# NickDrake117/GNNkeras

Measured on AMD Instinct MI355X. Metric: node-state updates/s (arcs x iterations / s), forward Loop, higher is better.
Workload: dtype f32; 1 GPU; C4 Erdos-Renyi 1000000 nodes / 10000000 arcs, state_dim=64, max_iteration=50, threshold=0 (k=50), node-focused, average aggregation, BN+Dense(159->64,selu) state net

## Files before the change

### gnnkeras_amd/csrc/gnnloop.hip

```cpp
#include <hip/hip_runtime.h>
#include <stdarg.h>
#include <stddef.h>
#include <stdio.h>
#include <stdlib.h>
#include <string.h>
#include <algorithm>
#include <mutex>
#include <string>
#include <vector>

#include "../../include/gnnloop.h"
#include "kernels_general.hpp"
#include "kernel_state_fused2.hpp"
#include "kernel_state_fused4.hpp"
#include "kernel_state_small.hpp"
#include "kernel_state_mid.hpp"
#include "kernel_state_lds.hpp"
#include "kernel_state_lds_types.hpp"
#include "kernel_state_wide.hpp"
#include "kernels_batch.hpp"
#include "kernels_setup.hpp"
#include "kernel_rowdense.hpp"
#include "kernel_state_xwide.hpp"

// ... 32 lines not shown
int state_ld(int S) {
    if (S <= 128) {
        int p = 16;
        while (p < S) p <<= 1;
        return p;
    }
    return round_up(S, 4);
}

struct Knobs {
    int pin;
    int flag_pin, env_pin;
    int mid_max_nodes;
    bool prefix_fusion, xwide, rowdense;
    bool xc; int xc_min_nodes;
};
const Knobs &process_knobs() {
    static const Knobs once = [] {
        Knobs k = {};
        const char *e;
        k.env_pin = (e = getenv("GNN_FUSED_KERNEL")) ? atoi(e) : 0;
        k.mid_max_nodes = (e = getenv("GNN_MID_MAX_NODES")) ? atoi(e) : 36000;
        k.prefix_fusion = !((e = getenv("GNN_PREFIX_FUSION")) && e[0] == '0');
        k.xwide = !((e = getenv("GNN_XWIDE")) && atoi(e) == 0);
        k.rowdense = !((e = getenv("GNN_ROWDENSE")) && e[0] == '0');
        return k;
    }();
    return once;
}
Knobs knobs(int flags) {
    Knobs k = process_knobs();
    k.flag_pin = (flags & GNN_FLAG_FUSED_GEN_MASK) >> 4;
    k.pin = k.flag_pin ? k.flag_pin : k.env_pin;
    const char *e = getenv("GNN_XC"), *m = getenv("GNN_XC_MIN_NODES");
    k.xc = !(e && atoi(e) == 0);
    k.xc_min_nodes = m ? atoi(m) : 196608;
    return k;
}

struct Carver {
    char *base;
    size_t off = 0;
    explicit Carver(void *b) : base((char *)b) {}
    template <typename T>
    T *take(size_t count) {
        off = (off + 255) & ~(size_t)255;
        T *p = base ? (T *)(base + off) : nullptr;
        off += count * sizeof(T);
        return p;
    }
};
// ... 306 lines not shown
    int count;
    float *Wf, *bf;
    float *Wc;
    int wrow_state, wrow_agg;
    gnn::Seg cseg[GNN_MAX_SEGS];
    int ncseg;
};

struct Plan {
    int N, E, S, SP, L, A, T;
    int H1max, Hmax_state, Hmax_out, Tout, M, G;
    bool composite, fused;
    int n_heavy;
    TypePlan tp[GNN_MAX_TYPES];
    int *flags;
    int *mid_bar;
    gnn::GroupTab gt;
    int n_groups;
    int group_tiles;
    int group_max_nodes;
    int *d_group_tabs;
    unsigned long long *set_bar;
    bool has_sets;
    int *pred0;
    int *tbeg;
    int *err;
    float *agg_arcs, *agg_nodes; int ld_agg_nodes;
    float *C; int ldC;
    float *Xc;
    float *Wx;
// ... 102 lines not shown
            TRY(check_csr(a.nodegraph, "nodegraph", a.nodegraph.n_dst, p.M));
        }
        if (a.n_heavy_segments > 0) {
            if (!a.heavy_seg_beg || !a.heavy_seg_end) return fail("heavy_seg_beg / heavy_seg_end is NULL");
            TRY(check_csr(a.adjacency_light, "adjacency_light", p.N, (a.nodes_src ? a.adjacency.n_src : p.N) + a.n_heavy_segments));
        }
        if (p.composite) {
            if (!a.type_nodes && p.N > 0) return fail("type_nodes is NULL");
            if (a.type_offsets[0] != 0 || a.type_offsets[p.T] != p.N) return fail("type_offsets must span [0, n_nodes]");
            for (int t = 0; t < p.T; ++t)
                TRY(check_csr(a.composite_adjacency[t], "composite_adjacency", p.N, a.nodes_src ? a.adjacency.n_src : p.N));
        }
    }

    Carver c(ws);
    p.flags = c.take<int>(a.max_iteration + GNN_LOOP_WORDS);
    p.err = p.flags ? p.flags + a.max_iteration + 12 : nullptr;
    p.mid_bar = p.flags ? p.flags + ((a.max_iteration + 16 + 31) & ~31) : nullptr;
    p.pred0 = c.take<int>(std::max(GNN_SMALL_MAX_TILES, p.group_tiles));
    p.d_group_tabs = c.take<int>(a.n_groups > 0 ? 4 * ((size_t)a.n_groups + 1) : 0);
    p.set_bar = c.take<unsigned long long>(a.n_groups > 0 ? 2 * (size_t)a.n_groups : 0);
    for (int t = 0; t < p.T; ++t) {
        p.tp[t].Wf = c.take<float>((size_t)a.net_state[t].in_dim * a.net_state[t].units[0]);
        p.tp[t].bf = c.take<float>(a.net_state[t].units[0]);
    }
    p.Wf_out = c.take<float>((size_t)a.net_output.in_dim * a.net_output.units[0]);
    p.bf_out = c.take<float>(a.net_output.units[0]);
    p.agg_arcs = c.take<float>((size_t)p.N * std::max(p.A, 1));
    p.ld_agg_nodes = p.composite ? sum_dt : (a.state_dim > 0 ? p.L : 0);
    p.agg_nodes = c.take<float>((size_t)p.N * std::max(p.ld_agg_nodes, 1));
    p.ldC = (p.H1max + 3) & ~3;
// ... 40 lines not shown
                if (p.A > 0) tp.cseg[tp.ncseg++] = gnn::Seg{p.agg_arcs, nullptr, p.A, p.A, 2 * p.S};
            }
        } else {
            const int dt = a.type_dim_label[t];
            tp.rows = a.type_nodes ? a.type_nodes + a.type_offsets[t] : nullptr;
            tp.count = a.type_offsets[t + 1] - a.type_offsets[t];
            tp.wrow_state = dt; tp.wrow_agg = dt + p.S;
            if (dt > 0) tp.cseg[tp.ncseg++] = gnn::Seg{a.nodes, tp.rows, a.ld_nodes, dt, 0};
            if (sum_dt > 0) tp.cseg[tp.ncseg++] = gnn::Seg{p.agg_nodes, tp.rows, p.ld_agg_nodes, sum_dt, dt + 2 * p.S};
            if (p.A > 0) tp.cseg[tp.ncseg++] = gnn::Seg{p.agg_arcs, tp.rows, p.A, p.A, dt + 2 * p.S + sum_dt};
        }
    }
    return 0;
}

inline const gnn_csr_t &iter_adjacency(const gnn_loop_args_t &a, const Plan &p) { return p.n_heavy > 0 ? a.adjacency_light : a.adjacency; }

}
#include "loop_route.hpp"
namespace {

int launch_heavy(const gnn_loop_args_t &a, const Plan &p, const int *gate, const float *src, hipStream_t st) {
    if (p.n_heavy == 0) return 0;
    float *buf = const_cast<float *>(src);
    const int first_virtual = a.nodes_src ? a.adjacency.n_src : p.N;
    const int grid = std::min(p.n_heavy, 256 * 8);
    switch (p.SP) {
        case 16: gnn::k_heavy_segments<16><<<grid, 256, 0, st>>>(gate, a.heavy_seg_beg, a.heavy_seg_end, p.n_heavy, a.adjacency.src, a.adjacency.w, buf, first_virtual); break;
        case 32: gnn::k_heavy_segments<32><<<grid, 256, 0, st>>>(gate, a.heavy_seg_beg, a.heavy_seg_end, p.n_heavy, a.adjacency.src, a.adjacency.w, buf, first_virtual); break;
        case 64: gnn::k_heavy_segments<64><<<grid, 256, 0, st>>>(gate, a.heavy_seg_beg, a.heavy_seg_end, p.n_heavy, a.adjacency.src, a.adjacency.w, buf, first_virtual); break;
// ... 43 lines not shown
    LAUNCH_OK();
    return 0;
}
int check_xc_args(const gnn_loop_args_t &a) {
    if (!a.xc) return 0;
    if (((uintptr_t)a.xc & 255) != 0) return fail("xc must be 256-byte aligned");
    if (a.xc_mode != GNN_XC_FILL && a.xc_mode != GNN_XC_VALID) return fail("unknown xc_mode %d", a.xc_mode);
    return 0;
}

int setup_constants(const gnn_loop_args_t &a, const Plan &p, hipStream_t st, bool zero_loop_words = false, bool skip_c = false,
                    const GivenAgg *given = nullptr, bool xc_line = false, bool xc_valid = false) {
    FoldList fl;
    for (int t = 0; t < p.T; ++t) fl.add(a.net_state[t], p.tp[t].Wf, p.tp[t].bf);
    if (a.net_output.kernel[0]) fl.add(a.net_output, p.Wf_out, p.bf_out);
    if (zero_loop_words) { fl.fa.zero_a = p.flags; fl.fa.n_a = a.max_iteration + GNN_LOOP_WORDS; fl.fa.zero_b = a.k_out; fl.fa.n_b = 1; }
    TRY(launch_fold_list(fl, st));
    if (xc_line) {
        const TypePlan &tp = p.tp[0];
        if (!xc_valid) TRY(fill_constants_line(a, p.N, a.state_dim > 0 ? p.L : 0, p.A, p.Xc, st));
        gnn::PackSegs ps;
        memset(&ps, 0, sizeof(ps));
        ps.n = tp.ncseg;
        for (int s2 = 0; s2 < tp.ncseg && s2 < 3; ++s2) { ps.width[s2] = tp.cseg[s2].width; ps.wrow[s2] = tp.cseg[s2].wrow; }
        const int H = tp.net->units[0];
        gnn::k_pack_wc<<<cdiv(32 * H, 256), 256, 0, st>>>(tp.Wf, tp.bf, H, ps, tp.Wc);
        LAUNCH_OK();
        return 0;
    }
    if (given) {
        if (p.A > 0) TRY(launch_copy2d(nullptr, given->arcs, given->ld_arcs, p.agg_arcs, p.A, p.N, p.A, p.A, st));
// ... 53 lines not shown
    const int L = a.state_dim > 0 ? p.L : 0;
    sa.N = p.N; sa.n_tiles = p.group_tiles; sa.groups = p.gt;
    if (p.n_groups > GNN_MAX_GROUPS || (p.n_groups > 0 && p.gt.n == 0)) {
        sa.groups.d_node_begin = p.d_group_tabs; sa.groups.d_tile_begin = p.d_group_tabs + (p.n_groups + 1); sa.groups.n_dev = p.n_groups;
    }
    sa.nodes = a.nodes; sa.ld_nodes = a.ld_nodes; sa.L = L;
    sa.nodes_src = a.nodes_src ? a.nodes_src : a.nodes; sa.ld_nodes_src = a.nodes_src ? a.ld_nodes_src : a.ld_nodes;
    sa.adj = gnn::SetupCsr{a.adjacency.rowptr, a.adjacency.src, a.adjacency.w, a.adjacency.row_scale};
    sa.arc_labels = a.arc_labels; sa.ld_arcs = a.ld_arcs; sa.A = p.A;
    sa.arcnode = gnn::SetupCsr{a.arcnode.rowptr, a.arcnode.src, a.arcnode.w, a.arcnode.row_scale};
    if (a.state_dim > 0) { sa.row_nodes = p.S; sa.row_aggn = 2 * p.S + p.L; sa.row_agga = 2 * p.S + 2 * p.L; }
    else                 { sa.row_agga = 2 * p.S; }
    sa.C = p.C; sa.ldC = p.ldC;
    sa.state0 = a.state_dim > 0 ? a.state0 : a.nodes; sa.ld_s0 = a.state_dim > 0 ? p.S : a.ld_nodes;
    sa.S = p.S; sa.thr = a.state_threshold; sa.pred0 = p.pred0;
    sa.zero_a = p.flags; sa.n_a = a.max_iteration + GNN_LOOP_WORDS; sa.zero_b = a.k_out; sa.n_b = std::max(1, p.n_groups);
    gnn::k_setup_small<<<sa.n_tiles + 1, 256, gnn::setup_small_lds(sa.net.H, 2 * L + p.A, std::max(a.net_state[0].in_dim, a.net_output.in_dim)), st>>>(sa);
    LAUNCH_OK();
    return 0;
}

__global__ void k_fold_error(const int *err, float *k_out) {
    if (*err != 0) *k_out = -1.0e9f;
}

int launch_fold_error(const Plan &p, float *k_out, hipStream_t st) {
    if (!k_out || !p.err) return 0;
    k_fold_error<<<1, 1, 0, st>>>(p.err, k_out);
    LAUNCH_OK();
    return 0;
}
// ... 83 lines not shown
    r.nseg = 1;
    r.segs[0] = gnn::Seg{p.agg, nullptr, p.SP, (int)m.units[1], 0};
    r.M = p.N;
    r.hid[0] = p.hid[0]; r.hid[1] = p.hid[1]; r.ld_hid = p.ld_hid;
    r.Y = dst; r.ldy = p.SP;
    r.gate = gate;
    if (flag_next) { r.pred_old = src; r.ld_pred = p.SP; r.pred_thr = a.state_threshold; r.pred_flag = flag_next; r.pred_k = k_out; r.pred_kval = k_val; }
    TRY(run_mlp(r, st));
    if (flag_next && !r.pred_fused) TRY(launch_converge(gate, dst, src, p.N, p.S, p.SP, p.SP, a.state_threshold, flag_next, k_out, k_val, st));
    return 0;
}

int iteration_fused(const gnn_loop_args_t &a, const Plan &p, IterKernel kernel, const int *gate, int n_gate, int gate_stride,
                    const float *src, float *dst, int row_base, int *flag_next, float *k_out, float k_val,
                    hipStream_t st, const gnn_csr_t *adj_override = nullptr, const float *agg_init = nullptr,
                    const int *rows_override = nullptr, int count_override = 0, const gnn_peer_set_t *peers = nullptr) {
    TRY(launch_heavy(a, p, n_gate == 1 ? gate : nullptr, src, st));
    const gnn_csr_t &adj = adj_override ? *adj_override : iter_adjacency(a, p);
    gnn::Fused2Args fa;
    memset(&fa, 0, sizeof(fa));
    fill_fused_args(fa, a, p, adj);
    fa.gate = n_gate ? gate : nullptr; fa.n_gate = n_gate; fa.gate_stride = gate_stride;
    fa.state_in = src; fa.state_out = dst; fa.row_base = row_base; fa.err = p.err;
    if (rows_override && fa.n_types == 1) {
        fa.tp[0].rows = rows_override; fa.tp[0].count = count_override;
        if (count_override == 0) fa.n_types = 0;
    }
    fa.flag_next = flag_next;
    fa.k_out = k_out; fa.k_val = k_val;
    fa.agg_init = agg_init;
    if (peers) {
        if (peers->n_peers < 0 || peers->n_peers > GNN_MAX_PEERS) return fail("n_peers %d out of [0, %d]", peers->n_peers, GNN_MAX_PEERS);
        fa.n_peers = peers->n_peers;
        for (int i = 0; i < peers->n_peers; ++i) fa.peer_out[i] = peers->state_out_full[i];
    }
    if (p.xc_ok && !adj.w && (agg_init || size_generation(p, a.flags) == 4)) fa.Xc = p.Xc;
    if (fa.n_types == 0) {
        if (k_out) TRY(launch_converge(fa.gate, src, src, 0, p.S, p.SP, p.SP, a.state_threshold, flag_next, k_out, k_val, st));
        return 0;
    }
    if (fa.n_peers > 0 && (p.SP == 128 || p.T != 1 || adj.w || a.net_state[0].n_layers != 1 || (p.SP != 32 && p.SP != 64) || p.n_heavy != 0))
        return fail("peer stores: homogeneous one-layer shards without per-arc weights or hub rows, state widths 17 .. 64");
    if (kernel == IterKernel::wide) FUSED_OK(gnn::launch_wide(fa, device_cus(), st, 0));
    else if (kernel == IterKernel::fused4 || agg_init || fa.n_peers > 0) FUSED_OK(gnn::launch_fused4(fa, p.SP, device_cus(), st));
    else FUSED_OK(gnn::launch_fused2(fa, p.SP, 8, device_cus(), st));
// ... 224 lines not shown
        for (int t = 0; t <= GNN_MAX_TYPES; ++t) to.off[t] = a.type_offsets[std::min(t, p.T)];
        gnn::k_group_type_begin<<<cdiv(p.T * (p.n_groups + 1), 256), 256, 0, st>>>(a.type_nodes, to, p.T, p.d_group_tabs, p.n_groups, p.tbeg);
        LAUNCH_OK();
        gnn::k_pred0_groups<<<p.n_groups, 256, 0, st>>>(p.d_group_tabs, a.state_dim > 0 ? a.state0 : a.nodes, a.state_dim > 0 ? p.S : a.ld_nodes, p.S,
                                                        a.state_threshold, p.pred0);
        LAUNCH_OK();
        if (a.ev_loop_begin) HIP_OK(hipEventRecord((hipEvent_t)a.ev_loop_begin, st));
        const int rc = loop_lds_types(a, p, st);
        if (rc != 0) return rc == 2 ? fail("LDS-resident loop kernel does not cover these convergence groups") : 1;
        if (a.ev_loop_end) HIP_OK(hipEventRecord((hipEvent_t)a.ev_loop_end, st));
        return output_stage(a, p, st);
    }
    default: break;
    }
    const bool small_setup = route.small_setup, xc_loop = route.xc_loop, xc_line = route.xc_line;
    if (xc_line && a.xc) { TRY(check_xc_args(a)); p.Xc = a.xc; }
    if (small_setup) TRY(setup_small(a, p, st));
    else             TRY(setup_constants(a, p, st, true, xc_loop, nullptr, xc_line,
                                         xc_line && a.xc && a.xc_mode == GNN_XC_VALID));

    const float *first = p.buf[0];
    if (a.state_dim > 0 && p.S == p.SP && p.n_heavy == 0 && (reinterpret_cast<uintptr_t>(a.state0) & 15) == 0) first = a.state0;
    else if (a.state_dim > 0) TRY(launch_copy2d(nullptr, a.state0, p.S, p.buf[0], p.SP, p.N, p.S, p.SP, st));
    else                      TRY(launch_copy2d(nullptr, a.nodes, a.ld_nodes, p.buf[0], p.SP, p.N, p.S, p.SP, st));
    if (p.SP != p.S) HIP_OK(hipMemsetAsync(p.buf[1], 0, sizeof(float) * (size_t)p.N * p.SP, st));
    if (!small_setup) TRY(launch_converge(nullptr, first, nullptr, p.N, p.S, p.SP, 0, a.state_threshold, p.flags, nullptr, 0.f, st));

    const IterKernel kernel = route.iter.kernel;
    if (kernel == IterKernel::xwide) TRY(setup_xwide(a, p, st));
    const bool no_exit = (a.flags & GNN_FLAG_NO_EARLY_EXIT) != 0;
// ... 5 lines not shown
    if (route.whole == WholeLoop::small) {
        persistent = loop_whole(a, p, false, first, B, small_setup ? p.pred0 : nullptr, small_setup ? p.group_tiles : 0, a.state_out, st);
        if (persistent == 1) return 1;
        if (persistent == 2 && small_setup) return fail("whole-loop kernel refused a graph its set-up kernel accepted");
    }
    bool loop_done = persistent == 0;
    if (!loop_done && route.try_mid) {
        const int rc = loop_whole(a, p, true, first, B, nullptr, 0, nullptr, st);
        if (rc == 1) return 1;
        loop_done = rc == 0;
    }
    for (int it = 0; !loop_done && it < a.max_iteration; ++it) {
        const int *gate = no_exit ? nullptr : p.flags + it;
        const float *src = it == 0 ? first : B[it & 1];
        float *dst = B[(it + 1) & 1];
        if (route.iter.fused())                  TRY(iteration_fused(a, p, kernel, gate, gate ? 1 : 0, 0, src, dst, 0, p.flags + it + 1, a.k_out, (float)(it + 1), st));
        else if (kernel == IterKernel::prefix)   TRY(iteration_prefix(a, p, gate, src, dst, p.flags + it + 1, a.k_out, (float)(it + 1), st));
        else if (kernel == IterKernel::xwide)    TRY(iteration_xwide(a, p, gate, src, dst, p.flags + it + 1, a.k_out, (float)(it + 1), st));
        else                                     TRY(iteration_unfused(a, p, gate, src, dst, 0, p.flags + it + 1, a.k_out, (float)(it + 1), st));
    }

    if (a.ev_loop_end) HIP_OK(hipEventRecord((hipEvent_t)a.ev_loop_end, st));

    if (persistent != 0) {
        const long total = (long)p.N * p.S;
        if (total > 0) {
            gnn::k_select_state<<<std::min(cdiv(total, 256), 256 * 16), 256, 0, st>>>(a.k_out, first, B[0], B[1], p.SP, a.state_out, p.S, p.N, p.S);
            LAUNCH_OK();
        }
    }
    TRY(output_stage(a, p, st));
// ... 433 lines not shown
```

### gnnkeras_amd/csrc/kernel_state_fused2.hpp

```cpp
#pragma once
#include <hip/hip_runtime.h>
#include "kernels_general.hpp"

namespace gnn {

struct FusedType {
    const int *rows;
    int count;
    const float *Wf;
    int wrow_state, wrow_agg;
    int H, act;
    const float *W2;
    const float *b2;
    int act2;
    const float *Wc;
    int out2;
};

struct Fused2Args {
    const int *gate; int n_gate, gate_stride;
    const int *rowptr, *src;
    const float *w, *row_scale;
    const float *state_in;
    float *state_out;
    int row_base;
    const float *C; int ldC;
    int n_types;
    FusedType tp[GNN_MAX_TYPES];
    int blk_begin[GNN_MAX_TYPES + 1];
    int S;
    float thr;
    int *flag_next;
    float *k_out; float k_val;
    int *err;
    const float *Xc;
    const float *agg_init;
    const void *hdr; void *hdr_write;
    float *peer_out[GNN_MAX_PEERS]; int n_peers;
};

inline char *last_kernel_name() { static thread_local char name[96] = ""; return name; }
#define GNN_SET_KERNEL_NAME(...) snprintf(::gnn::last_kernel_name(), 96, __VA_ARGS__)

template <int SP, int TM, int NW>
struct Fused2Cfg {
    static constexpr int NT = 64 * NW;
    static constexpr int LPR = SP / 4;
    static constexpr int NPP = NT / LPR;
    static constexpr int NPASS = TM / NPP;
    static constexpr int IPL = 16 / LPR;
    static constexpr int LDX = 2 * SP + 2;
    static constexpr bool SWZ = SP >= 32;
    static constexpr int LDW = SWZ ? SP : SP + 32;
// ... 319 lines not shown
```

### gnnkeras_amd/csrc/kernel_state_fused4.hpp

```cpp
#pragma once
#include <hip/hip_runtime.h>
#include "kernel_state_fused2.hpp"
#include "buffer_ops.hpp"

namespace gnn {

constexpr int XC_K = 32;

template <int SP, int NC = 4, bool L2 = false, bool XC = false, int VPL = 1>
struct Fused4Cfg {
    static constexpr int NW = 16, NT = 64 * NW;
    static constexpr int NCONS = NC;
    static constexpr int NPROD = NW - NCONS;
    static constexpr int LPR = SP / (4 * VPL);
    static constexpr int RPWV = 64 / LPR;
    static constexpr int PPT = 16 / RPWV;
    static constexpr int IPL = 16 / LPR;
    static constexpr int LDX = 2 * SP + 2;
    static constexpr bool SWZ = SP >= 32;
    static constexpr int LDW = SWZ ? SP : SP + 32;
    static constexpr int NCT = SP / 16;
    static constexpr int NS = SP == 64 ? (L2 ? 3 : (XC ? 4 : 5)) : 8;
    static constexpr int WROWS = 2 * SP + (XC ? XC_K : 0);
    static constexpr int SLOT = 16 * LDX;
    static constexpr int W2F = L2 ? SP * LDW + SP : 0;
    static constexpr size_t LDS_BYTES = sizeof(float) * ((size_t)NS * SLOT + WROWS * LDW + W2F) + sizeof(int) * 2 * NS;
};

__device__ __forceinline__ void activate4(int act, f32x4 &x) {
#define F4_ALL(expr)                                        \
    _Pragma("unroll") for (int e = 0; e < 4; ++e) {         \
        const float v = x[e];                               \
        x[e] = (expr);                                      \
    }
    switch (act) {
        case GNN_ACT_RELU: F4_ALL(fmaxf(v, 0.0f)) break;
        case GNN_ACT_SELU: F4_ALL(v > 0.0f ? 1.0507009873554805f * v : (1.0507009873554805f * 1.6732632423543772f) * (expf(v) - 1.0f)) break;
        case GNN_ACT_TANH: F4_ALL(tanhf(v)) break;
        case GNN_ACT_SIGMOID: F4_ALL(1.0f / (1.0f + expf(-v))) break;
        case GNN_ACT_ELU: F4_ALL(v > 0.0f ? v : expf(v) - 1.0f) break;
        case GNN_ACT_SOFTPLUS: F4_ALL(v > 20.0f ? v : log1pf(expf(v))) break;
// ... 27 lines not shown
    int open = a.gate == nullptr;
    for (int i = 0; i < a.n_gate; ++i) open |= a.gate[(size_t)i * a.gate_stride] != 0;
    using Cfg = Fused4Cfg<SP, NC, L2, XC, VPL>;
    constexpr int NT = Cfg::NT, LPR = Cfg::LPR, IPL = Cfg::IPL, LDX = Cfg::LDX, LDW = Cfg::LDW, NS = Cfg::NS;
#ifndef GNN_F4_SPIN_MAX
#define GNN_F4_SPIN_MAX (1 << 22)
#endif
    constexpr int SPIN_MAX = GNN_F4_SPIN_MAX;
    int bad = 0;
    extern __shared__ __attribute__((aligned(16))) char smem[];
    float *Xs = reinterpret_cast<float *>(smem);
    float *Ws = Xs + NS * Cfg::SLOT;
    float *W2s = Ws + Cfg::WROWS * LDW;
    int *fill = reinterpret_cast<int *>(W2s + Cfg::W2F);
    int *freed = fill + NS;

    const int tid = threadIdx.x, lane = tid & 63, wave = tid >> 6;
    if (tid == 0) F4_STAMP(0);
    const int S = a.S;
    int ty = 0;
    while (ty + 1 < a.n_types && (int)blockIdx.x >= a.blk_begin[ty + 1]) ++ty;
    const FusedType tp = a.tp[ty];
    const int O2 = tp.out2 > 0 ? tp.out2 : S;
    const int bid = blockIdx.x - a.blk_begin[ty], nblk = a.blk_begin[ty + 1] - a.blk_begin[ty];
    const int count = tp.count;
    const int *__restrict__ rows = tp.rows;

    const int ntiles = (count + 15) / 16;
    const int xcd = bid & 7, lb = bid >> 3;
    const int blk_per_xcd = (nblk + 7 - xcd) >> 3;
    const int tpx = (ntiles + 7) >> 3;
    const int t_end = min(ntiles, (xcd + 1) * tpx);
    const int t_first = xcd * tpx + lb;
    const int T = t_first < t_end ? (t_end - t_first + blk_per_xcd - 1) / blk_per_xcd : 0;

    const __amdgpu_buffer_rsrc_t r_C = buf_rsrc(XC ? a.Xc : a.C), r_rows = buf_rsrc(tp.rows), r_state = buf_rsrc(a.state_in),
                                 r_rowptr = buf_rsrc(a.rowptr), r_src = buf_rsrc(a.src), r_w = buf_rsrc(HAS_W ? a.w : nullptr),
                                 r_scale = buf_rsrc(a.row_scale), r_init = buf_rsrc(INIT ? a.agg_init : nullptr);
    const bool has_scale = a.row_scale != nullptr;
    char *__restrict__ obase = reinterpret_cast<char *>(a.state_out);
    int any = 0;

    const int p = wave - Cfg::NCONS;
    const int qr = lane / LPR;
    const int l4 = lane % LPR;
    const int njobs = T * Cfg::PPT;
    auto job_m = [&](int n) -> int {
        const int m = (t_first + (n / Cfg::PPT) * blk_per_xcd) * 16 + (n % Cfg::PPT) * Cfg::RPWV + qr;
        return (n < njobs && m < count) ? m : -1;
    };
    auto node_of = [&](int m) -> int {
        const int jr = buf_ld_i32(r_rows, m >= 0 ? 4u * (unsigned)m : BUF_OFF);
        return m >= 0 ? (rows ? jr : m) : -1;
    };
    int jA = -1, jB = -1, begA = 0, endA = 0;
    int idsA[IPL]; float wsA[IPL];
#pragma unroll
    for (int u = 0; u < IPL; ++u) { idsA[u] = 0; wsA[u] = 0.0f; }
    if (wave >= Cfg::NCONS) {
        jA = node_of(job_m(p)); jB = node_of(job_m(p + Cfg::NPROD));
        if (HDR && a.hdr) {
            const u32x4 h = __builtin_amdgcn_raw_buffer_load_b128(buf_rsrc(a.hdr), (int)((((unsigned)blockIdx.x * Cfg::NPROD + (unsigned)p) * 64u + (unsigned)lane) * 16u), 0, 0);
            begA = (int)h[0]; endA = (int)h[1]; idsA[0] = (int)h[2];
            if (IPL > 1) idsA[IPL > 1 ? 1 : 0] = (int)h[3];
        } else {
        begA = buf_ld_i32(r_rowptr, jA >= 0 ? 4u * (unsigned)jA : BUF_OFF);
        endA = buf_ld_i32(r_rowptr, jA >= 0 ? 4u * (unsigned)jA + 4u : BUF_OFF);
#pragma unroll
        for (int u = 0; u < IPL; ++u) {
            const int e = begA + u * LPR + l4;
            idsA[u] = buf_ld_i32(r_src, e < endA ? 4u * (unsigned)e : BUF_OFF);
            wsA[u] = HAS_W ? buf_ld_f32(r_w, e < endA ? 4u * (unsigned)e : BUF_OFF) : 0.0f;
        }
        }
        if (HDR && a.hdr_write) {
// ... 26 lines not shown
            if (n < tp.H) v = tp.Wc[(size_t)(k - 2 * SP) * tp.H + n];
        } else {
            const int kk = k < SP ? k : k - SP;
            if (kk < S && n < tp.H) v = tp.Wf[(size_t)((k < SP ? tp.wrow_state : tp.wrow_agg) + kk) * tp.H + n];
        }
        Ws[k * LDW + (Cfg::SWZ ? (n ^ ((k & 1) << 4)) : n)] = v;
    }
    if (L2) {
        for (int i = tid; i < SP * SP; i += NT) {
            const int k = i / SP, n = i % SP;
            W2s[k * LDW + (Cfg::SWZ ? (n ^ ((k & 1) << 4)) : n)] = (k < tp.H && n < O2) ? tp.W2[(size_t)k * O2 + n] : 0.0f;
        }
        if (tid < SP) W2s[SP * LDW + tid] = tid < O2 ? tp.b2[tid] : 0.0f;
    }
    if (tid < 2 * NS) fill[tid] = 0;
    __syncthreads();
    if (!open) return;
    if (tid == 0) F4_STAMP(1);

    if (wave >= Cfg::NCONS) {
#ifdef GNN_F4_PROFILE
        const unsigned long long tr_ = f4_now();
#endif
        for (int n = p; n < njobs; n += Cfg::NPROD) {
            const int t = n / Cfg::PPT;
            const int row = (n % Cfg::PPT) * Cfg::RPWV + qr;
            const int j = jA;
#ifdef GNN_F4_PROFILE
            unsigned long long tg_ = f4_now();
#endif
            const int begB = buf_ld_i32(r_rowptr, jB >= 0 ? 4u * (unsigned)jB : BUF_OFF);
            const int endB = buf_ld_i32(r_rowptr, jB >= 0 ? 4u * (unsigned)jB + 4u : BUF_OFF);
            const int jC = node_of(job_m(n + 2 * Cfg::NPROD));
            const float scl = buf_ld_f32(r_scale, j >= 0 ? 4u * (unsigned)j : BUF_OFF);
            f32x4 own[VPL], acc[VPL];
#pragma unroll
            for (int x = 0; x < VPL; ++x) {
                own[x] = buf_ld_f32x4(r_state, j >= 0 ? (unsigned)(a.row_base + j) * (unsigned)(SP * 4) + 16u * (unsigned)(VPL * l4 + x) : BUF_OFF);
                acc[x] = (f32x4){0.f, 0.f, 0.f, 0.f};
                if (INIT) acc[x] = buf_ld_f32x4(r_init, j >= 0 ? (unsigned)j * (unsigned)(SP * 4) + 16u * (unsigned)(VPL * l4 + x) : BUF_OFF);
            }
            int idsB[IPL]; float wsB[IPL];
            int rem = endA - begA, eb = begA;
            int idc[IPL]; float wsc[IPL];
#pragma unroll
            for (int u = 0; u < IPL; ++u) { idc[u] = idsA[u]; wsc[u] = wsA[u]; }
            bool first = true;
#pragma unroll 1
// ... 69 lines not shown
                *reinterpret_cast<float2 *>(xr + SP) = make_float2(acc[x][0], acc[x][1]);
                *reinterpret_cast<float2 *>(xr + SP + 2) = make_float2(acc[x][2], acc[x][3]);
            }
            if (l4 == 0) Xs[s * Cfg::SLOT + row * LDX + 2 * SP] = __int_as_float(j);
            if (lane == 0) __hip_atomic_fetch_add(&fill[s], 1, __ATOMIC_RELEASE, __HIP_MEMORY_SCOPE_WORKGROUP);
            if (n == p && p == 0 && lane == 0) F4_STAMP(2);
        }
#ifdef GNN_F4_PROFILE
        if (lane == 0) atomicAdd(&g_f4_prof[6], f4_now() - tr_);
#endif
    } else {
        const int r = lane & 15, g = lane >> 4;
#ifdef GNN_F4_PROFILE
        const unsigned long long tr_ = f4_now();
#endif
        for (int t = wave; t < T; t += Cfg::NCONS) {
            f32x4 c[Cfg::NCT];
            float xa[XC ? XC_K / 4 : 1];
            if (XC) {
                const int m = (t_first + t * blk_per_xcd) * 16 + r;
                const int jr = buf_ld_i32(r_rows, m < count ? 4u * (unsigned)m : BUF_OFF);
                const int jx = m < count ? (rows ? jr : m) : -1;
#pragma unroll
                for (int q = 0; q < XC_K / 4; ++q)
                    xa[q] = buf_ld_f32(r_C, jx >= 0 ? ((unsigned)jx * (unsigned)XC_K + (unsigned)(4 * q + g)) * 4u : BUF_OFF);
#pragma unroll
                for (int ci = 0; ci < Cfg::NCT; ++ci) c[ci] = (f32x4){0.f, 0.f, 0.f, 0.f};
            } else {
                int jrow[4];
#pragma unroll
                for (int reg = 0; reg < 4; ++reg) {
                    const int m = (t_first + t * blk_per_xcd) * 16 + 4 * g + reg;
                    const int jr = buf_ld_i32(r_rows, m < count ? 4u * (unsigned)m : BUF_OFF);
                    jrow[reg] = m < count ? (rows ? jr : m) : -1;
                }
#pragma unroll
                for (int ci = 0; ci < Cfg::NCT; ++ci) {
                    const int col = 16 * ci + r;
#pragma unroll
                    for (int reg = 0; reg < 4; ++reg)
                        c[ci][reg] = buf_ld_f32(r_C, (jrow[reg] >= 0 && col < tp.H) ? ((unsigned)jrow[reg] * (unsigned)a.ldC + (unsigned)col) * 4u : BUF_OFF);
                }
            }
            const int s = t % NS, round = t / NS;
#ifdef GNN_F4_PROFILE
            unsigned long long tc_ = f4_now();
#endif
// ... 229 lines not shown
```

### gnnkeras_amd/csrc/loop_route.hpp

```cpp
#pragma once

namespace {

enum class WholeLoop { none, lds, lds_types, small, mid };
enum class IterKernel { unfused, fused2, fused4, wide, prefix, xwide };

struct IterRoute {
    IterKernel kernel;
    int fuse;
    bool split_ok;
    bool fused() const { return kernel == IterKernel::fused2 || kernel == IterKernel::fused4 || kernel == IterKernel::wide; }
};

struct LoopRoute {
    WholeLoop whole;
    bool small_setup;
    bool try_mid;
    IterRoute iter;
    bool xc_loop;
    bool xc_line;
    const char *refused;
};

bool state_softmax(const gnn_loop_args_t &a, const Plan &p) {
    for (int t = 0; t < p.T; ++t)
        if (a.net_state[t].n_layers >= 1 && a.net_state[t].activation[a.net_state[t].n_layers - 1] == GNN_ACT_SOFTMAX) return true;
    return false;
}

int fuse_class(const gnn_loop_args_t &a, const Plan &p) {
    if ((a.flags & GNN_FLAG_UNFUSED) || p.SP > 128) return 0;
    if ((size_t)(std::max(a.adjacency.n_src, p.N) + p.n_heavy) * p.SP * 4 >= ((size_t)1 << 32) || (size_t)p.N * p.ldC * 4 >= ((size_t)1 << 32)) return 0;
    if ((size_t)iter_adjacency(a, p).nnz * 4 >= ((size_t)1 << 32) || ((size_t)p.N + 1) * 4 >= ((size_t)1 << 32)) return 0;
    bool two = false;
    for (int t = 0; t < p.T; ++t) {
// ... 99 lines not shown
        return r;
    }
    const bool soft = state_softmax(a, p);
    const bool small = fz != 0 && !soft && small_covers(a, p, k);
    r.small_setup = small && setup_small_covers(a, p);
    r.try_mid = !r.small_setup && fz == 1 && !soft && mid_covers(a, p, k);
    r.whole = small ? WholeLoop::small : r.try_mid ? WholeLoop::mid : WholeLoop::none;
    if (p.has_sets) r.refused = "convergence group sets need the one-CU-per-group form (gnn_loop_groups_supported() != 2 for these args)";
    else if (p.n_groups > GNN_MAX_GROUPS)
        r.refused = "more than " GNN_ROUTE_STR(GNN_MAX_GROUPS) " convergence groups need every group to fit one CU's LDS (gnn_loop_groups_supported() != 2)";
    else if (p.n_groups > 0 && !r.small_setup) r.refused = "convergence groups need the whole-loop kernel (gnn_loop_groups_supported() == 0 for these args)";
    if (r.refused) return r;
    r.xc_loop = p.xc_ok && !small && fz == 1 && !r.try_mid && p.SP != 128 && !iter_adjacency(a, p).w &&
                r.iter.kernel == IterKernel::fused4 && size_generation(p, a.flags) == 4;
    r.xc_line = r.xc_loop && !p.composite && p.N > 0;
    return r;
}

void route_name(const LoopRoute &r, char *name, size_t n) {
    static const char *const stem[] = {"k_aggregate_vec", "k_state_fused2", "k_state_fused4", "k_state_wide", "k_state_fused4<.., L2>", "k_state_xwide_b3"};
    if (r.refused) snprintf(name, n, "refused: %s", r.refused);
    else if (r.whole == WholeLoop::lds) snprintf(name, n, "k_state_lds");
    else if (r.whole == WholeLoop::lds_types) snprintf(name, n, "k_state_lds_types");
    else if (r.small_setup) snprintf(name, n, "k_state_small(setup_small)");
    else snprintf(name, n, "%s%s%s%s", r.whole == WholeLoop::small ? "k_state_small > " : "", r.try_mid ? "k_state_mid > " : "",
                  stem[(int)r.iter.kernel], r.xc_loop ? "+xc" : "");
}

}
```

Measured before the change: 21.80 billion arc-updates/s.

## Add dynamic tile queue with atomic ticket draws to fused4 state kernel

Replaces the purely static per-XCD tile partition in the fused4 iteration kernel with a hybrid scheme. About three quarters of each block's tiles stay statically assigned, and the remainder are drawn dynamically from per-iteration, per-range global atomic counters through an LDS ticket ring shared by producer and consumer waves. The aim is to cut load imbalance across blocks caused by irregular Erdos-Renyi degrees. The cost is extra atomics, spin-waits, LDS use and more complex producer/consumer coordination. It is enabled by default only for large tile counts.

Result: no change. 21.93 billion arc-updates/s, median of 6 (+0.6%).

```diff
diff --git a/gnnkeras_amd/csrc/gnnloop.hip b/gnnkeras_amd/csrc/gnnloop.hip
--- a/gnnkeras_amd/csrc/gnnloop.hip
+++ b/gnnkeras_amd/csrc/gnnloop.hip
@@ -70,6 +70,7 @@
     int mid_max_nodes;
     bool prefix_fusion, xwide, rowdense;
     bool xc; int xc_min_nodes;
+    int tile_queue;
 };
 const Knobs &process_knobs() {
     static const Knobs once = [] {
@@ -91,6 +92,7 @@
     const char *e = getenv("GNN_XC"), *m = getenv("GNN_XC_MIN_NODES");
     k.xc = !(e && atoi(e) == 0);
     k.xc_min_nodes = m ? atoi(m) : 196608;
+    k.tile_queue = (e = getenv("GNN_F4_TILE_QUEUE")) ? atoi(e) : 1;
     return k;
 }
 
@@ -427,6 +429,8 @@
     int n_heavy;
     TypePlan tp[GNN_MAX_TYPES];
     int *flags;
+    int *tq; long tq_ints;
+    bool tq_on;
     int *mid_bar;
     gnn::GroupTab gt;
     int n_groups;
@@ -559,7 +563,11 @@
     }
 
     Carver c(ws);
-    p.flags = c.take<int>(a.max_iteration + GNN_LOOP_WORDS);
+    p.tq_ints = (p.SP <= 64 && !(a.flags & GNN_FLAG_UNFUSED) && a.n_groups == 0 && a.max_iteration > 0) ? gnn::tq_counter_ints(a.max_iteration, p.T) : 0;
+    p.tq_on = false;
+    const size_t loop_words = round_up(a.max_iteration + GNN_LOOP_WORDS, 32);
+    p.flags = c.take<int>(loop_words + (size_t)p.tq_ints);
+    p.tq = (p.flags && p.tq_ints > 0) ? p.flags + loop_words : nullptr;
     p.err = p.flags ? p.flags + a.max_iteration + 12 : nullptr;
     p.mid_bar = p.flags ? p.flags + ((a.max_iteration + 16 + 31) & ~31) : nullptr;
     p.pred0 = c.take<int>(std::max(GNN_SMALL_MAX_TILES, p.group_tiles));
@@ -630,6 +638,10 @@
     return 0;
 }
 
+inline int zeroed_loop_words(const gnn_loop_args_t &a, const Plan &p) {
+    return p.tq_on ? (int)(p.tq - p.flags + p.tq_ints) : a.max_iteration + GNN_LOOP_WORDS;
+}
+
 inline const gnn_csr_t &iter_adjacency(const gnn_loop_args_t &a, const Plan &p) { return p.n_heavy > 0 ? a.adjacency_light : a.adjacency; }
 
 }
@@ -703,7 +715,7 @@
     FoldList fl;
     for (int t = 0; t < p.T; ++t) fl.add(a.net_state[t], p.tp[t].Wf, p.tp[t].bf);
     if (a.net_output.kernel[0]) fl.add(a.net_output, p.Wf_out, p.bf_out);
-    if (zero_loop_words) { fl.fa.zero_a = p.flags; fl.fa.n_a = a.max_iteration + GNN_LOOP_WORDS; fl.fa.zero_b = a.k_out; fl.fa.n_b = 1; }
+    if (zero_loop_words) { fl.fa.zero_a = p.flags; fl.fa.n_a = zeroed_loop_words(a, p); fl.fa.zero_b = a.k_out; fl.fa.n_b = 1; }
     TRY(launch_fold_list(fl, st));
     if (xc_line) {
         const TypePlan &tp = p.tp[0];
@@ -787,7 +799,7 @@
     sa.C = p.C; sa.ldC = p.ldC;
     sa.state0 = a.state_dim > 0 ? a.state0 : a.nodes; sa.ld_s0 = a.state_dim > 0 ? p.S : a.ld_nodes;
     sa.S = p.S; sa.thr = a.state_threshold; sa.pred0 = p.pred0;
-    sa.zero_a = p.flags; sa.n_a = a.max_iteration + GNN_LOOP_WORDS; sa.zero_b = a.k_out; sa.n_b = std::max(1, p.n_groups);
+    sa.zero_a = p.flags; sa.n_a = zeroed_loop_words(a, p); sa.zero_b = a.k_out; sa.n_b = std::max(1, p.n_groups);
     gnn::k_setup_small<<<sa.n_tiles + 1, 256, gnn::setup_small_lds(sa.net.H, 2 * L + p.A, std::max(a.net_state[0].in_dim, a.net_output.in_dim)), st>>>(sa);
     LAUNCH_OK();
     return 0;
@@ -901,7 +913,7 @@
 int iteration_fused(const gnn_loop_args_t &a, const Plan &p, IterKernel kernel, const int *gate, int n_gate, int gate_stride,
                     const float *src, float *dst, int row_base, int *flag_next, float *k_out, float k_val,
                     hipStream_t st, const gnn_csr_t *adj_override = nullptr, const float *agg_init = nullptr,
-                    const int *rows_override = nullptr, int count_override = 0, const gnn_peer_set_t *peers = nullptr) {
+                    const int *rows_override = nullptr, int count_override = 0, const gnn_peer_set_t *peers = nullptr, int *tile_counters = nullptr) {
     TRY(launch_heavy(a, p, n_gate == 1 ? gate : nullptr, src, st));
     const gnn_csr_t &adj = adj_override ? *adj_override : iter_adjacency(a, p);
     gnn::Fused2Args fa;
@@ -916,6 +928,7 @@
     fa.flag_next = flag_next;
     fa.k_out = k_out; fa.k_val = k_val;
     fa.agg_init = agg_init;
+    fa.tq = tile_counters;
     if (peers) {
         if (peers->n_peers < 0 || peers->n_peers > GNN_MAX_PEERS) return fail("n_peers %d out of [0, %d]", peers->n_peers, GNN_MAX_PEERS);
         fa.n_peers = peers->n_peers;
@@ -1170,6 +1183,7 @@
     default: break;
     }
     const bool small_setup = route.small_setup, xc_loop = route.xc_loop, xc_line = route.xc_line;
+    p.tq_on = route.tile_queue;
     if (xc_line && a.xc) { TRY(check_xc_args(a)); p.Xc = a.xc; }
     if (small_setup) TRY(setup_small(a, p, st));
     else             TRY(setup_constants(a, p, st, true, xc_loop, nullptr, xc_line,
@@ -1205,7 +1219,8 @@
         const int *gate = no_exit ? nullptr : p.flags + it;
         const float *src = it == 0 ? first : B[it & 1];
         float *dst = B[(it + 1) & 1];
-        if (route.iter.fused())                  TRY(iteration_fused(a, p, kernel, gate, gate ? 1 : 0, 0, src, dst, 0, p.flags + it + 1, a.k_out, (float)(it + 1), st));
+        if (route.iter.fused())                  TRY(iteration_fused(a, p, kernel, gate, gate ? 1 : 0, 0, src, dst, 0, p.flags + it + 1, a.k_out, (float)(it + 1), st,
+                                                                     nullptr, nullptr, nullptr, 0, nullptr, route.tile_queue ? p.tq + gnn::tq_counter(it, p.T, 0, 0) : nullptr));
         else if (kernel == IterKernel::prefix)   TRY(iteration_prefix(a, p, gate, src, dst, p.flags + it + 1, a.k_out, (float)(it + 1), st));
         else if (kernel == IterKernel::xwide)    TRY(iteration_xwide(a, p, gate, src, dst, p.flags + it + 1, a.k_out, (float)(it + 1), st));
         else                                     TRY(iteration_unfused(a, p, gate, src, dst, 0, p.flags + it + 1, a.k_out, (float)(it + 1), st));
diff --git a/gnnkeras_amd/csrc/kernel_state_fused2.hpp b/gnnkeras_amd/csrc/kernel_state_fused2.hpp
--- a/gnnkeras_amd/csrc/kernel_state_fused2.hpp
+++ b/gnnkeras_amd/csrc/kernel_state_fused2.hpp
@@ -37,6 +37,7 @@
     const float *agg_init;
     const void *hdr; void *hdr_write;
     float *peer_out[GNN_MAX_PEERS]; int n_peers;
+    int *tq;
 };
 
 inline char *last_kernel_name() { static thread_local char name[96] = ""; return name; }
diff --git a/gnnkeras_amd/csrc/kernel_state_fused4.hpp b/gnnkeras_amd/csrc/kernel_state_fused4.hpp
--- a/gnnkeras_amd/csrc/kernel_state_fused4.hpp
+++ b/gnnkeras_amd/csrc/kernel_state_fused4.hpp
@@ -2,6 +2,7 @@
 #include <hip/hip_runtime.h>
 #include "kernel_state_fused2.hpp"
 #include "buffer_ops.hpp"
+#include "tile_queue.hpp"
 
 namespace gnn {
 
@@ -24,7 +25,10 @@
     static constexpr int WROWS = 2 * SP + (XC ? XC_K : 0);
     static constexpr int SLOT = 16 * LDX;
     static constexpr int W2F = L2 ? SP * LDW + SP : 0;
-    static constexpr size_t LDS_BYTES = sizeof(float) * ((size_t)NS * SLOT + WROWS * LDW + W2F) + sizeof(int) * 2 * NS;
+    static constexpr int PRO = 3 * NPROD / PPT;
+    static constexpr int AHEAD = (PRO + NS + 4 + 3) & ~3;
+    static_assert(AHEAD <= 64 && AHEAD + NCONS + NS <= TQ_RING, "the ticket ring is too short for this look-ahead");
+    static constexpr size_t LDS_BYTES = sizeof(float) * ((size_t)NS * SLOT + WROWS * LDW + W2F) + sizeof(int) * (2 * NS + 2 + TQ_RING);
 };
 
 __device__ __forceinline__ void activate4(int act, f32x4 &x) {
@@ -82,6 +86,9 @@
     float *W2s = Ws + Cfg::WROWS * LDW;
     int *fill = reinterpret_cast<int *>(W2s + Cfg::W2F);
     int *freed = fill + NS;
+    int *tq_drawn = freed + NS;
+    int *tq_end = tq_drawn + 1;
+    int *tq_map = tq_end + 1;
 
     const int tid = threadIdx.x, lane = tid & 63, wave = tid >> 6;
     if (tid == 0) F4_STAMP(0);
@@ -95,12 +102,24 @@
     const int *__restrict__ rows = tp.rows;
 
     const int ntiles = (count + 15) / 16;
-    const int xcd = bid & 7, lb = bid >> 3;
-    const int blk_per_xcd = (nblk + 7 - xcd) >> 3;
-    const int tpx = (ntiles + 7) >> 3;
-    const int t_end = min(ntiles, (xcd + 1) * tpx);
-    const int t_first = xcd * tpx + lb;
-    const int T = t_first < t_end ? (t_end - t_first + blk_per_xcd - 1) / blk_per_xcd : 0;
+    const TileRange tr = tq_range(ntiles, nblk, bid, a.tq != nullptr, Cfg::PRO);
+    const int tdyn = tq_first_dynamic(tr, Cfg::PRO);
+    const bool dynq = a.tq != nullptr && tr.dyn_lo < tr.hi;
+    int *const tq_cnt = a.tq + tq_counter(0, a.n_types, ty, tr.x);
+    int T = dynq ? TQ_OPEN : tr.nstatic;
+    auto tile_static = [&](int t) -> int { return t < tr.nstatic ? tq_static_tile(tr, t) : ntiles; };
+    auto tile_of = [&](int t_) -> int {
+        const int t = __builtin_amdgcn_readfirstlane(t_);
+        if (!dynq || t < tdyn) return tile_static(t);
+        int spin = 0;
+        while (__builtin_amdgcn_readfirstlane(f4_ld_acquire(tq_drawn)) <= t) {
+            if (spin >= SPIN_MAX) { bad = 1; T = 0; return ntiles; }
+            ++spin; __builtin_amdgcn_s_sleep(1);
+        }
+        const int te = __builtin_amdgcn_readfirstlane(__hip_atomic_load(tq_end, __ATOMIC_RELAXED, __HIP_MEMORY_SCOPE_WORKGROUP));
+        if (t >= te) { T = te; return ntiles; }
+        return __builtin_amdgcn_readfirstlane(__hip_atomic_load(&tq_map[t & (TQ_RING - 1)], __ATOMIC_RELAXED, __HIP_MEMORY_SCOPE_WORKGROUP));
+    };
 
     const __amdgpu_buffer_rsrc_t r_C = buf_rsrc(XC ? a.Xc : a.C), r_rows = buf_rsrc(tp.rows), r_state = buf_rsrc(a.state_in),
                                  r_rowptr = buf_rsrc(a.rowptr), r_src = buf_rsrc(a.src), r_w = buf_rsrc(HAS_W ? a.w : nullptr),
@@ -112,10 +131,9 @@
     const int p = wave - Cfg::NCONS;
     const int qr = lane / LPR;
     const int l4 = lane % LPR;
-    const int njobs = T * Cfg::PPT;
-    auto job_m = [&](int n) -> int {
-        const int m = (t_first + (n / Cfg::PPT) * blk_per_xcd) * 16 + (n % Cfg::PPT) * Cfg::RPWV + qr;
-        return (n < njobs && m < count) ? m : -1;
+    auto job_m = [&](int n, int tile) -> int {
+        const int m = tile * 16 + (n % Cfg::PPT) * Cfg::RPWV + qr;
+        return m < count ? m : -1;
     };
     auto node_of = [&](int m) -> int {
         const int jr = buf_ld_i32(r_rows, m >= 0 ? 4u * (unsigned)m : BUF_OFF);
@@ -126,7 +144,8 @@
 #pragma unroll
     for (int u = 0; u < IPL; ++u) { idsA[u] = 0; wsA[u] = 0.0f; }
     if (wave >= Cfg::NCONS) {
-        jA = node_of(job_m(p)); jB = node_of(job_m(p + Cfg::NPROD));
+        jA = node_of(job_m(p, tile_static(p / Cfg::PPT)));
+        jB = node_of(job_m(p + Cfg::NPROD, tile_static((p + Cfg::NPROD) / Cfg::PPT)));
         if (HDR && a.hdr) {
             const u32x4 h = __builtin_amdgcn_raw_buffer_load_b128(buf_rsrc(a.hdr), (int)((((unsigned)blockIdx.x * Cfg::NPROD + (unsigned)p) * 64u + (unsigned)lane) * 16u), 0, 0);
             begA = (int)h[0]; endA = (int)h[1]; idsA[0] = (int)h[2];
@@ -183,6 +202,8 @@
         if (tid < SP) W2s[SP * LDW + tid] = tid < O2 ? tp.b2[tid] : 0.0f;
     }
     if (tid < 2 * NS) fill[tid] = 0;
+    if (tid == 2 * NS) *tq_drawn = tdyn;
+    if (tid == 2 * NS + 1) *tq_end = TQ_OPEN;
     __syncthreads();
     if (!open) return;
     if (tid == 0) F4_STAMP(1);
@@ -191,7 +212,7 @@
 #ifdef GNN_F4_PROFILE
         const unsigned long long tr_ = f4_now();
 #endif
-        for (int n = p; n < njobs; n += Cfg::NPROD) {
+        for (int n = p; n < T * Cfg::PPT; n += Cfg::NPROD) {
             const int t = n / Cfg::PPT;
             const int row = (n % Cfg::PPT) * Cfg::RPWV + qr;
             const int j = jA;
@@ -200,7 +221,7 @@
 #endif
             const int begB = buf_ld_i32(r_rowptr, jB >= 0 ? 4u * (unsigned)jB : BUF_OFF);
             const int endB = buf_ld_i32(r_rowptr, jB >= 0 ? 4u * (unsigned)jB + 4u : BUF_OFF);
-            const int jC = node_of(job_m(n + 2 * Cfg::NPROD));
+            const int jC = node_of(job_m(n + 2 * Cfg::NPROD, tile_of((n + 2 * Cfg::NPROD) / Cfg::PPT)));
             const float scl = buf_ld_f32(r_scale, j >= 0 ? 4u * (unsigned)j : BUF_OFF);
             f32x4 own[VPL], acc[VPL];
 #pragma unroll
@@ -300,11 +321,40 @@
 #ifdef GNN_F4_PROFILE
         const unsigned long long tr_ = f4_now();
 #endif
+        const bool drawer = dynq && __builtin_amdgcn_readfirstlane(wave) == 0;
+        bool ended = false;
+        auto draw = [&](int tb, int nl) {
+            const int lt = tb + lane, u = lt - TQ_RING;
+            int k = 0;
+            if (lane < nl) k = __hip_atomic_fetch_add(tq_cnt, 1, __ATOMIC_RELAXED, __HIP_MEMORY_SCOPE_AGENT);
+            const int g = tq_ticket_tile(tr, k, ntiles);
+            int spin = 0;
+            while (__any(lane < nl && u >= tdyn && f4_ld_acquire(&freed[max(u, 0) % NS]) < u / NS + 1)) {
+                if (spin >= SPIN_MAX) { bad = 1; break; }
+                ++spin; __builtin_amdgcn_s_sleep(1);
+            }
+            if (lane < nl) tq_map[lt & (TQ_RING - 1)] = g;
+            const unsigned long long valid = __ballot(lane < nl && g < ntiles), dry = __ballot(lane < nl && g >= ntiles);
+            if (dry || bad) {
+                ended = true;
+                if (lane == 0) {
+                    __hip_atomic_store(tq_end, bad ? 0 : tb + (valid ? 64 - __builtin_clzll(valid) : 0), __ATOMIC_RELAXED, __HIP_MEMORY_SCOPE_WORKGROUP);
+                    __hip_atomic_store(tq_drawn, 0x7fffffff, __ATOMIC_RELEASE, __HIP_MEMORY_SCOPE_WORKGROUP);
+                }
+            } else if (lane == 0) __hip_atomic_store(tq_drawn, tb + nl, __ATOMIC_RELEASE, __HIP_MEMORY_SCOPE_WORKGROUP);
+        };
+        if (drawer && tdyn < Cfg::AHEAD) draw(tdyn, Cfg::AHEAD - tdyn);
         for (int t = wave; t < T; t += Cfg::NCONS) {
+            if (drawer && !ended && t + Cfg::AHEAD + Cfg::NCONS > tdyn) {
+                const int tb = max(t + Cfg::AHEAD, tdyn);
+                draw(tb, t + Cfg::AHEAD + Cfg::NCONS - tb);
+            }
+            const int tile = tile_of(t);
+            if (bad || t >= T) break;
             f32x4 c[Cfg::NCT];
             float xa[XC ? XC_K / 4 : 1];
             if (XC) {
-                const int m = (t_first + t * blk_per_xcd) * 16 + r;
+                const int m = tile * 16 + r;
                 const int jr = buf_ld_i32(r_rows, m < count ? 4u * (unsigned)m : BUF_OFF);
                 const int jx = m < count ? (rows ? jr : m) : -1;
 #pragma unroll
@@ -316,7 +366,7 @@
                 int jrow[4];
 #pragma unroll
                 for (int reg = 0; reg < 4; ++reg) {
-                    const int m = (t_first + t * blk_per_xcd) * 16 + 4 * g + reg;
+                    const int m = tile * 16 + 4 * g + reg;
                     const int jr = buf_ld_i32(r_rows, m < count ? 4u * (unsigned)m : BUF_OFF);
                     jrow[reg] = m < count ? (rows ? jr : m) : -1;
                 }
diff --git a/gnnkeras_amd/csrc/loop_route.hpp b/gnnkeras_amd/csrc/loop_route.hpp
--- a/gnnkeras_amd/csrc/loop_route.hpp
+++ b/gnnkeras_amd/csrc/loop_route.hpp
@@ -19,6 +19,7 @@
     IterRoute iter;
     bool xc_loop;
     bool xc_line;
+    bool tile_queue;
     const char *refused;
 };
 
@@ -148,6 +149,10 @@
     r.xc_loop = p.xc_ok && !small && fz == 1 && !r.try_mid && p.SP != 128 && !iter_adjacency(a, p).w &&
                 r.iter.kernel == IterKernel::fused4 && size_generation(p, a.flags) == 4;
     r.xc_line = r.xc_loop && !p.composite && p.N > 0;
+    long tiles = 0;
+    for (int t = 0; t < p.T; ++t) tiles += (p.tp[t].count + 15) / 16;
+    r.tile_queue = k.tile_queue != 0 && r.iter.kernel == IterKernel::fused4 && !r.small_setup && p.tq_ints > 0 &&
+                   (k.tile_queue == 2 || tiles >= 100L * 2 * device_cus());
     return r;
 }
 
diff --git a/gnnkeras_amd/csrc/tile_queue.hpp b/gnnkeras_amd/csrc/tile_queue.hpp
--- /dev/null
+++ b/gnnkeras_amd/csrc/tile_queue.hpp
@@ -0,0 +1,56 @@
+#pragma once
+
+#ifndef __HIP__
+#ifndef __host__
+#define __host__
+#define __device__
+#endif
+#endif
+
+namespace gnn {
+
+constexpr int TQ_RANGES = 8;
+constexpr int TQ_LINE = 32;
+constexpr int TQ_RING = 64;
+constexpr int TQ_OPEN = 1 << 24;
+
+struct TileRange {
+    int x;
+    int lo, hi;
+    int lb, nb;
+    int nstatic;
+    int dyn_lo;
+};
+
+__host__ __device__ inline TileRange tq_range(int ntiles, int nblk, int bid, bool queue, int pro) {
+    TileRange r;
+    const int nx = nblk < TQ_RANGES ? (nblk > 0 ? nblk : 1) : TQ_RANGES;
+    const int x = r.x = bid % nx;
+    const int tpx = (ntiles + nx - 1) / nx;
+    r.lb = bid / nx;
+    r.nb = (nblk + nx - 1 - x) / nx;
+    r.lo = x * tpx < ntiles ? x * tpx : ntiles;
+    r.hi = (x + 1) * tpx < ntiles ? (x + 1) * tpx : ntiles;
+    const int len = r.hi - r.lo;
+    if (!queue) {
+        r.nstatic = r.lb < len ? (len - r.lb + r.nb - 1) / r.nb : 0;
+        r.dyn_lo = r.hi;
+        return r;
+    }
+    const int share = len / r.nb;
+    const int want = 3 * share / 4 > pro ? 3 * share / 4 : pro;
+    r.nstatic = share < want ? share : want;
+    r.dyn_lo = r.lo + r.nstatic * r.nb;
+    return r;
+}
+
+__host__ __device__ inline int tq_static_tile(const TileRange &r, int t) { return r.lo + r.lb + t * r.nb; }
+
+__host__ __device__ inline int tq_ticket_tile(const TileRange &r, int k, int none) { return k < r.hi - r.dyn_lo ? r.dyn_lo + k : none; }
+
+__host__ __device__ inline int tq_first_dynamic(const TileRange &r, int pro) { return r.nstatic > pro ? r.nstatic : pro; }
+
+__host__ __device__ inline long tq_counter(int it, int n_types, int ty, int x) { return (((long)it * n_types + ty) * TQ_RANGES + x) * TQ_LINE; }
+__host__ __device__ inline long tq_counter_ints(int n_launches, int n_types) { return tq_counter(n_launches, n_types, 0, 0); }
+
+}
```
